# vvvwo/KSS-ICP

Measured on AMD Instinct MI355X. Metric: icp_iterations_per_sec, higher is better.
Workload: dtype f32; 1 GPU; C2: one 100000x100000 uniform-sphere pair per GPU, 50 fixed ICP iterations + fitness pass per step (exact NN + cov reduce + host 3x3 SVD), R_z(10deg), jitter 1e-3; n_src=100000, n_tgt=100000, pairs_per_gpu=1, nn_engine=cell list + brute-force fallback, nn_arithmetic=reference (no fma)

## Files before the change

### kss-icp_amd/csrc/kss_api.hip

```cpp
#pragma clang fp contract(off)

#include "kss_ctx.hpp"

extern "C" {

int kss_version(void) { return KSS_VERSION; }

const char* kss_status_string(int s) {
    switch (s) {
        case KSS_OK: return "ok";
        case KSS_ERR_ARG: return "invalid argument";
        case KSS_ERR_HIP: return "HIP runtime error";
        case KSS_ERR_NOMEM: return "out of memory";
        case KSS_ERR_NODEVICE: return "no usable GPU device";
        case KSS_ERR_CAPACITY: return "output buffer too small";
        case KSS_ERR_RCCL: return "RCCL error";
        case KSS_ERR_DEGENERATE: return "degenerate point-to-plane system";
        default: return "unknown status";
    }
}

const char* kss_last_error(const kss_ctx* ctx) { return ctx ? ctx->err.c_str() : ""; }

static int ctx_create_common(int device_id, void* stream, bool borrow, kss_ctx** out) {
// ... 5 lines not shown
    if (hipSetDevice(device_id) != hipSuccess) return KSS_ERR_NODEVICE;
    kss_ctx* c = new (std::nothrow) kss_ctx();
    if (!c) return KSS_ERR_NOMEM;
    c->device = device_id;
    if (borrow) {
        c->stream = (hipStream_t)stream;
        c->own_stream = false;
    } else {
        if (hipStreamCreateWithFlags(&c->stream, hipStreamNonBlocking) != hipSuccess) { delete c; return KSS_ERR_HIP; }
        c->own_stream = true;
    }
    kss_live_contexts().fetch_add(1);
    static std::atomic<unsigned long long> ctx_serial{0};
    c->seq = (ctx_serial.fetch_add(1) + 1ull) << 40;
    *out = c;
    return KSS_OK;
}

int kss_ctx_create(int device_id, kss_ctx** out) { return ctx_create_common(device_id, nullptr, false, out); }
int kss_ctx_create_on_stream(int device_id, void* hip_stream, kss_ctx** out) {
    return ctx_create_common(device_id, hip_stream, true, out);
}

int kss_ctx_destroy(kss_ctx* c) {
    if (!c) return KSS_ERR_ARG;
    hipSetDevice(c->device);
    hipStreamSynchronize(c->stream);
    prof_collect(c);
    for (auto& ep : c->ev_pool) { hipEventDestroy(ep.a); hipEventDestroy(ep.b); }
    c->ev_pool.clear();
    DevBuf* bufs[] = {&c->tgt4, &c->src0, &c->cur[0], &c->cur[1], &c->keys, &c->partials, &c->sums, &c->nn_work,
                      &c->red_work, &c->pair_red, &c->state, &c->cs, &c->scratch_a, &c->scratch_b, &c->scratch_c,
                      &c->stage_src, &c->stage_tgt, &c->stage_idx, &c->stage_d2, &c->stage_out, &c->g_counts, &c->g_start,
                      &c->g_cursor, &c->g_bsums, &c->g_sorted, &c->g_list, &c->g_count, &c->g_bbox, &c->g_partials, &c->g_start2, &c->g_pairs, &c->g_stamps, &c->g_pos, &c->g_nnst, &c->res_pos, &c->res_wc, &c->res_perm, &c->pack_seg, &c->reg_s, &c->reg_t, &c->reg_p, &c->reg_all, &c->reg_f, &c->reg_g, &c->oct_pts, &c->oct_cen, &c->oct_a, &c->oct_b, &c->oct_tmp, &c->pre_partials, &c->pre_state, &c->g_rowpair, &c->g_gate, &c->p2l_idx, &c->p2l_d2, &c->p2l_perm, &c->p2l_rows, &c->p2l_nrm, &c->p2l_n64, &c->trim_rows, &c->trim_state};
    for (DevBuf* b : bufs)
        if (b->p) hipFree(b->p);
    if (c->h_sums) hipHostFree(c->h_sums);
    if (c->h_seq) hipHostFree(c->h_seq);
    if (c->h_p2l) hipHostFree(c->h_p2l);
    if (c->h_box) hipHostFree(c->h_box);
    if (c->h_xf) hipHostFree(c->h_xf);
    if (c->gate_bar) hipFree(c->gate_bar);
    if (c->res_gate) hipFree(c->res_gate);
    if (c->bar_state) hipFree(c->bar_state);
    if (c->h_state) hipHostFree(c->h_state);
    for (kss_ctx* w : c->workers) kss_ctx_destroy(w);
    c->workers.clear();
    if (c->own_stream) hipStreamDestroy(c->stream);
    kss_live_contexts().fetch_sub(1);
    delete c;
    return KSS_OK;
}

int kss_ctx_synchronize(kss_ctx* c) {
    if (!c) return KSS_ERR_ARG;
    HIPCHK(c, hipStreamSynchronize(c->stream));
    return KSS_OK;
}

void* kss_ctx_stream(kss_ctx* c) { return c ? (void*)c->stream : nullptr; }

int kss_ctx_set_nn_mode(kss_ctx* c, int nn_mode) {
    if (!c || nn_mode < KSS_NN_AUTO || nn_mode > KSS_NN_GRID) return KSS_ERR_ARG;
    c->nn_mode = nn_mode;
    return KSS_OK;
}

// ... 1034 lines not shown
```

### kss-icp_amd/csrc/kss_ctx.hpp

```cpp
#pragma once
#include <dlfcn.h>
#include <hip/hip_runtime.h>

#include <algorithm>
#include <atomic>
#include <chrono>
#include <cmath>
#include <cstdio>
#include <cstdlib>
#include <cstring>
#include <mutex>
#include <string>
#include <thread>
#include <vector>

#include "kss_internal.hpp"
#include "kss_host_pool.hpp"

using namespace kss;

struct DevBuf {
    void* p = nullptr;
    size_t cap = 0;
};

struct kss_ctx {
    int device = 0;
    int cu_count = 0;
    hipStream_t stream = nullptr;
    bool own_stream = false;
    std::string err;
    int nn_mode = KSS_NN_AUTO;
    double grid_stats[8] = {0, 0, 0, 0, 0, 0, 0, 0};
    double last_setup_ms = 0, last_loop_ms = 0;
    double t_launch_us = 0, t_wait_us = 0, t_host_us = 0;
    bool timing = false;
    bool tables_staged = false;
    int64_t stats_ns = -1, stats_nt = -1;

    DevBuf tgt4, src0, cur[2], keys, partials, sums, nn_work, red_work, pair_red, state, cs, scratch_a,
        scratch_b, scratch_c, stage_src, stage_tgt, stage_idx, stage_d2, stage_out, g_counts, g_start, g_cursor,
        g_bsums, g_sorted, g_list, g_count, g_bbox, g_partials, g_start2, g_pairs, g_stamps, g_pos, g_nnst, res_pos, res_wc, res_perm, pack_seg, reg_s, reg_t, reg_p, reg_all, reg_f, reg_g, oct_pts, oct_cen, oct_a, oct_b, oct_tmp, pre_partials, pre_state, g_rowpair, g_gate;
    DevBuf p2l_idx, p2l_d2, p2l_perm, p2l_rows, p2l_nrm, p2l_n64;
    DevBuf trim_rows, trim_state;
    HostPool pool;
    std::vector<kss_ctx*> workers;
    std::vector<unsigned long long> last_stamps;
    int stamps_nblk = 0; unsigned long long stamps_seq = 0;
    std::vector<float> h_bbox;
    unsigned int* h_box = nullptr; unsigned int* h_box_dev = nullptr; size_t h_box_bytes = 0;
    unsigned box_tag = 0; int box_rows = 0;
    double evals_sum = 0.0, evals_launches = 0.0;
    void* h_sums = nullptr;  size_t h_sums_cap = 0;
    void* h_sums_dev = nullptr;
    void* h_p2l = nullptr; size_t h_p2l_cap = 0;
    void* h_p2l_dev = nullptr;
    unsigned long long* h_seq = nullptr;
    unsigned long long* h_seq_dev = nullptr;
    size_t h_seq_bytes = 0;
    struct Gated {
        int supported = -1;
        bool want_next = false;
        bool pending = false;
        bool chain = false;
        int steps_left = 0;
        int max_steps = 1;
        int slot = 0;
        unsigned long long seq = 0;
        int32_t stamp = 0;
        const void* d_in = nullptr; void* d_out = nullptr;
        bool fma = false, full = false, want_full = false; double max_d2 = 0.0;
    } gated;
    bool ws_dirty = false;
    bool defer_wait = false;
    PairState* h_xf = nullptr; PairState* h_xf_dev = nullptr;
// ... 148 lines not shown
```

### kss-icp_amd/csrc/kss_engine.hip

```cpp
#pragma clang fp contract(off)

#include <emmintrin.h>

#include "kss_ctx.hpp"

namespace kss {

static int restore_zero_at_rest(kss_ctx* c);
static bool resident_gate_available(kss_ctx* c, int npairs);

static int resident_rows_limit(kss_ctx* c) {
    if (c->cu_count <= 0) {
        hipDeviceProp_t prop;
        c->cu_count = hipGetDeviceProperties(&prop, c->device) == hipSuccess && prop.multiProcessorCount > 0 ? prop.multiProcessorCount : 1;
        (void)hipGetLastError();
    }
    return c->cu_count;
}

constexpr int PUB_PAIRS = 32;
static int ensure_pub(kss_ctx* c, int npairs = PUB_PAIRS);

struct PairGeom {
    int64_t ns, nt;
// ... 298 lines not shown
                for (int k = 0; k < 3; ++k) { if (g & 1) mx[k] = std::max(mx[k], f[k]); else mn[k] = std::min(mn[k], f[k]); }
                ++g;
                continue;
            }
            __builtin_ia32_pause();
            if ((spin & 4095) == 4095 && std::chrono::duration<double, std::milli>(std::chrono::steady_clock::now() - t0).count() > 20.0) break;
        }
        have_box = g == 2 * nbb;
        if (!have_box) { for (int k = 0; k < 3; ++k) { mn[k] = INFINITY; mx[k] = -INFINITY; } }
    }
    if (!have_box) {
        std::vector<float>& hb = c->h_bbox;
        hb.resize((size_t)nbb * 6);
        HIPCHK(c, hipMemcpyAsync(hb.data(), c->g_bbox.p, hb.size() * sizeof(float), hipMemcpyDeviceToHost, c->stream));
        HIPCHK(c, hipStreamSynchronize(c->stream));
        for (int b = 0; b < nbb; ++b)
            for (int k = 0; k < 3; ++k) { mn[k] = std::min(mn[k], hb[(size_t)b * 6 + k]); mx[k] = std::max(mx[k], hb[(size_t)b * 6 + 3 + k]); }
    }
    if (!(std::isfinite(mn[0]) && std::isfinite(mn[1]) && std::isfinite(mn[2]) && std::isfinite(mx[0]) && std::isfinite(mx[1]) && std::isfinite(mx[2])))
        return set_err(c, KSS_ERR_ARG, "non-finite target coordinates");
    GridParams gp;
    choose_cells(mn, mx, nt, gp);
    pl.gp = gp;
    const size_t ncells = (size_t)gp.gx * gp.gy * gp.gz;
    KCHK(ensure_zeroed(c, c->g_counts, 2 * ncells * sizeof(int32_t)));
    KCHK(ensure(c, c->g_start, (2 * ncells + 8) * sizeof(int32_t)));
    KCHK(ensure(c, c->g_bsums, scan_scratch_bytes((int)(2 * ncells))));
    KCHK(ensure(c, c->g_sorted, (size_t)nt * sizeof(float4)));
    KCHK(ensure(c, c->g_list, (size_t)ns * sizeof(int32_t)));
    KCHK(ensure(c, c->g_pos, (size_t)ns * sizeof(float4)));
    c->nn_have = false;
    KCHK(ensure(c, c->g_nnst, (size_t)ns * sizeof(float2)));
    KCHK(ensure_zeroed(c, c->g_count, 64));
    if (getenv("KSS_COUNTS_CHECK")) {
        HIPCHK(c, hipStreamSynchronize(c->stream));
        std::vector<int32_t> h(2 * ncells);
        HIPCHK(c, hipMemcpy(h.data(), c->g_counts.p, h.size() * sizeof(int32_t), hipMemcpyDeviceToHost));
        size_t bad = 0, first = 0;
        for (size_t k = 0; k < h.size(); ++k)
            if (h[k] != 0) { if (!bad) first = k; ++bad; }
        if (bad) {
            std::fprintf(stderr, "[kss] counts check: %zu cells x 2 (%d x %d x %d), buffer %zu bytes, %zu non-zero counters, first at %zu = %d\n", ncells,
                         gp.gx, gp.gy, gp.gz, c->g_counts.cap, bad, first, h[first]);
            return set_err(c, KSS_ERR_HIP, "cell counters not zero at rest");
        }
    }
    pl.gpairs[0].gp = gp;
    pl.gpairs[0].cell_base = 0;
    launch_grid_build_pair(c->stream, tgt, nt, (float4*)c->src0.p + g.src_base, ns, gp, (int32_t*)c->g_counts.p, (int32_t*)c->g_start.p + 1,
                           (int32_t*)c->g_bsums.p, (float4*)c->g_sorted.p, (float4*)c->cur[0].p);
    HIPCHK(c, hipGetLastError());
    c->grid_stats[0] = gp.h; c->grid_stats[1] = gp.gx; c->grid_stats[2] = gp.gy; c->grid_stats[3] = gp.gz;
    if (c->stats_ns != ns || c->stats_nt != nt) { c->grid_stats[4] = 0; c->grid_stats[5] = 0; }
    c->grid_stats[6] = ns; c->grid_stats[7] = nt;
    if (c->prof && (c->stats_ns != ns || c->stats_nt != nt)) {
        c->stats_ns = ns; c->stats_nt = nt;
        KCHK(ensure(c, c->scratch_c, 64));
        HIPCHK(c, hipMemsetAsync(c->scratch_c.p, 0, 16, c->stream));
        launch_grid_stats(c->stream, (const float4*)c->src0.p + g.src_base, ns, gp, (const int32_t*)c->g_start.p + 1, (unsigned long long*)c->scratch_c.p);
        unsigned long long hst[2] = {0, 0};
        HIPCHK(c, hipMemcpyAsync(hst, c->scratch_c.p, 16, hipMemcpyDeviceToHost, c->stream));
        HIPCHK(c, hipStreamSynchronize(c->stream));
        c->grid_stats[5] = (double)hst[0];
        c->grid_stats[4] = (double)hst[1];
    }
    return KSS_OK;
}

static int grid_setup_batch(kss_ctx* c, IcpPlan& pl) {
    if (!pl.gridb) return KSS_OK;
    const int np = pl.npairs;
    std::vector<GridPairDev>& hp = pl.gpairs;
    int64_t sum_nt = 0;
    for (int p = 0; p < np; ++p) sum_nt += pl.g[p].nt;
    ProfScope ps(c, KSS_K_GRID_BUILD);
    KCHK(ensure(c, c->g_pairs, (size_t)np * sizeof(GridPairDev)));
    KCHK(ensure(c, c->g_bbox, (size_t)np * 6 * sizeof(float)));
    HIPCHK(c, hipMemcpyAsync(c->g_pairs.p, hp.data(), (size_t)np * sizeof(GridPairDev), hipMemcpyHostToDevice, c->stream));
    launch_gridb_bbox(c->stream, (const float4*)c->tgt4.p, (const GridPairDev*)c->g_pairs.p, np, (float*)c->g_bbox.p);
    std::vector<float> hb((size_t)np * 6);
    HIPCHK(c, hipMemcpyAsync(hb.data(), c->g_bbox.p, hb.size() * sizeof(float), hipMemcpyDeviceToHost, c->stream));
    HIPCHK(c, hipStreamSynchronize(c->stream));
    int64_t cells = 0, sorted_base = 0;
// ... 1361 lines not shown
```

### kss-icp_amd/csrc/kss_grid.hip

```cpp
#pragma clang fp contract(off)

#include <hip/hip_runtime.h>

#include <cstring>

#include <rocprim/rocprim.hpp>

#include <cstdlib>

#include "kss_internal.hpp"
#include "kss_device.hpp"

namespace kss {

__global__ __launch_bounds__(256) void grid_count2_kernel(const float4* __restrict__ tgt, int nt, int nbt, const float4* __restrict__ src, int ns,
                                                          GridParams gp, int32_t* __restrict__ counts) {
    const bool is_src = (int)blockIdx.x >= nbt;
    const int i = ((int)blockIdx.x - (is_src ? nbt : 0)) * 256 + (int)threadIdx.x;
    if (i >= (is_src ? ns : nt)) return;
    const float4 p = is_src ? src[i] : tgt[i];
    const int cx = cell_coord(p.x, gp.ox, gp.inv_h, gp.gx), cy = cell_coord(p.y, gp.oy, gp.inv_h, gp.gy),
              cz = cell_coord(p.z, gp.oz, gp.inv_h, gp.gz);
    atomicAdd(&counts[(is_src ? gp.gx * gp.gy * gp.gz : 0) + (cz * gp.gy + cy) * gp.gx + cx], 1);
}

constexpr int SCAN_CHUNK = 4096;

__global__ __launch_bounds__(256) void scan_block_sums_kernel(const int32_t* __restrict__ in, int n, int32_t* __restrict__ block_sums) {
    __shared__ int sh[4];
    typedef int32_t int4u __attribute__((ext_vector_type(4), aligned(4)));
    const int base = blockIdx.x * SCAN_CHUNK;
    int s = 0;
#pragma unroll
    for (int k = 0; k < 4; ++k) {
        const int i = base + (k * 256 + (int)threadIdx.x) * 4;
        if (i + 3 < n) { const int4u v = *(const int4u*)(in + i); s += (v.x + v.y) + (v.z + v.w); }
        else { if (i < n) s += in[i]; if (i + 1 < n) s += in[i + 1]; if (i + 2 < n) s += in[i + 2]; }
    }
#pragma unroll
    for (int off = 32; off > 0; off >>= 1) s += __shfl_down(s, off, 64);
    if ((threadIdx.x & 63) == 0) sh[threadIdx.x >> 6] = s;
    __syncthreads();
    if (threadIdx.x == 0) block_sums[blockIdx.x] = sh[0] + sh[1] + sh[2] + sh[3];
}

__global__ __launch_bounds__(1024) void scan_of_block_sums_kernel(int32_t* __restrict__ block_sums, int nb) {
    __shared__ int wave_tot[16];
    const int tid = threadIdx.x, lane = tid & 63, wave = tid >> 6;
    const int per = (nb + 1023) / 1024;
    const int lo = min(tid * per, nb), hi = min(nb, lo + per);
    int s = 0;
    for (int i = lo; i < hi; ++i) s += block_sums[i];
    int incl = s;
#pragma unroll
    for (int off = 1; off < 64; off <<= 1) {
        const int v = __shfl_up(incl, off, 64);
        if (lane >= off) incl += v;
    }
    if (lane == 63) wave_tot[wave] = incl;
    __syncthreads();
    int run = incl - s;
    for (int w = 0; w < 16; ++w) run += w < wave ? wave_tot[w] : 0;
    for (int i = lo; i < hi; ++i) {
        const int v = block_sums[i];
        block_sums[i] = run;
        run += v;
    }
}

template <bool SELF>
__global__ __launch_bounds__(256) void scan_apply_kernel(const int32_t* __restrict__ in, int n, const int32_t* __restrict__ block_sums,
                                                         int32_t* __restrict__ out_start) {
    typedef int32_t int4u __attribute__((ext_vector_type(4), aligned(4)));
    __shared__ int sh_tot[4][4];
    __shared__ int sh_off[4];
    const int tid = threadIdx.x, lane = tid & 63, wave = tid >> 6;
    int offset = 0;
    if constexpr (SELF) {
        int part = 0;
        for (int b = tid; b < (int)blockIdx.x; b += 256) part += block_sums[b];
#pragma unroll
        for (int off = 32; off > 0; off >>= 1) part += __shfl_down(part, off, 64);
        if (lane == 0) sh_off[wave] = part;
    } else {
        offset = block_sums[blockIdx.x];
    }
    const int base = blockIdx.x * SCAN_CHUNK;
    int4u v[4];
    int incl[4];
#pragma unroll
    for (int k = 0; k < 4; ++k) {
        const int i = base + (k * 256 + tid) * 4;
        if (i + 3 < n) v[k] = *(const int4u*)(in + i);
        else { v[k].x = i < n ? in[i] : 0; v[k].y = i + 1 < n ? in[i + 1] : 0; v[k].z = i + 2 < n ? in[i + 2] : 0; v[k].w = 0; }
        int x = (v[k].x + v[k].y) + (v[k].z + v[k].w);
#pragma unroll
        for (int off = 1; off < 64; off <<= 1) {
            const int t = __shfl_up(x, off, 64);
            if (lane >= off) x += t;
        }
        incl[k] = x;
        if (lane == 63) sh_tot[k][wave] = x;
    }
    __syncthreads();
    if constexpr (SELF) offset = sh_off[0] + sh_off[1] + sh_off[2] + sh_off[3];
    int run = offset;
#pragma unroll
    for (int k = 0; k < 4; ++k) {
        int before = 0;
#pragma unroll
        for (int w = 0; w < 4; ++w) before += w < wave ? sh_tot[k][w] : 0;
        const int own = (v[k].x + v[k].y) + (v[k].z + v[k].w);
        const int r0 = run + before + (incl[k] - own);
        const int i = base + (k * 256 + tid) * 4;
        int4u o;
        o.x = r0; o.y = r0 + v[k].x; o.z = o.y + v[k].y; o.w = o.z + v[k].z;
        if (i + 3 < n) *(int4u*)(out_start + i) = o;
        else { if (i < n) out_start[i] = o.x; if (i + 1 < n) out_start[i + 1] = o.y; if (i + 2 < n) out_start[i + 2] = o.z; }
        if (i <= n - 1 && n - 1 <= i + 3) out_start[n] = o.x + (n - 1 >= i ? v[k].x : 0) + (n - 1 >= i + 1 ? v[k].y : 0) + (n - 1 >= i + 2 ? v[k].z : 0) + (n - 1 >= i + 3 ? v[k].w : 0);
        run += (sh_tot[k][0] + sh_tot[k][1]) + (sh_tot[k][2] + sh_tot[k][3]);
    }
}

using BigScanConfig = rocprim::scan_config<256, 64, rocprim::block_load_method::block_load_transpose, rocprim::block_store_method::block_store_transpose,
                                           rocprim::block_scan_algorithm::reduce_then_scan>;

size_t scan_scratch_bytes(int n) {
    size_t bytes = 0;
    if (rocprim::inclusive_scan<BigScanConfig>(nullptr, bytes, (const int32_t*)nullptr, (int32_t*)nullptr, (size_t)n, rocprim::plus<int32_t>(), (hipStream_t)0) != hipSuccess) bytes = 0;
    return std::max<size_t>(bytes, ((size_t)(n + SCAN_CHUNK - 1) / SCAN_CHUNK + 1) * sizeof(int32_t)) + 256;
}

static void launch_scan(hipStream_t st, const int32_t* d_counts, int ncells, int32_t* d_start, int32_t* d_scratch) {
    static const bool lib = getenv("KSS_SCAN_LIB") != nullptr;
    if (lib && ncells > 1024 * SCAN_CHUNK) {
        size_t bytes = 0;
        if (rocprim::inclusive_scan<BigScanConfig>(nullptr, bytes, d_counts, d_start + 1, (size_t)ncells, rocprim::plus<int32_t>(), st) == hipSuccess) {
            hipMemsetAsync(d_start, 0, sizeof(int32_t), st);
            if (rocprim::inclusive_scan<BigScanConfig>((void*)d_scratch, bytes, d_counts, d_start + 1, (size_t)ncells, rocprim::plus<int32_t>(), st) == hipSuccess) return;
        }
        (void)hipGetLastError();
    }
    int32_t* d_block_sums = d_scratch;
    const int nb = (ncells + SCAN_CHUNK - 1) / SCAN_CHUNK;
    hipLaunchKernelGGL(scan_block_sums_kernel, dim3(nb), dim3(256), 0, st, d_counts, ncells, d_block_sums);
    if (nb <= 1024) {
        hipLaunchKernelGGL(scan_apply_kernel<true>, dim3(nb), dim3(256), 0, st, d_counts, ncells, d_block_sums, d_start);
    } else {
        hipLaunchKernelGGL(scan_of_block_sums_kernel, dim3(1), dim3(1024), 0, st, d_block_sums, nb);
        hipLaunchKernelGGL(scan_apply_kernel<false>, dim3(nb), dim3(256), 0, st, d_counts, ncells, d_block_sums, d_start);
    }
}

__global__ __launch_bounds__(256) void grid_scatter2_kernel(const float4* __restrict__ tgt, int nt, int nbt, const float4* __restrict__ src, int ns,
                                                            GridParams gp, int32_t* __restrict__ counts, const int32_t* __restrict__ start,
                                                            float4* __restrict__ sorted, float4* __restrict__ src_tmp) {
    const bool is_src = (int)blockIdx.x >= nbt;
    const int i = ((int)blockIdx.x - (is_src ? nbt : 0)) * 256 + (int)threadIdx.x;
    if (i >= (is_src ? ns : nt)) return;
    float4 p = is_src ? src[i] : tgt[i];
    const int cx = cell_coord(p.x, gp.ox, gp.inv_h, gp.gx), cy = cell_coord(p.y, gp.oy, gp.inv_h, gp.gy),
              cz = cell_coord(p.z, gp.oz, gp.inv_h, gp.gz);
    const int cell = (is_src ? gp.gx * gp.gy * gp.gz : 0) + (cz * gp.gy + cy) * gp.gx + cx;
    const int pos = start[cell] + atomicSub(&counts[cell], 1) - 1 - (is_src ? nt : 0);
    p.w = __int_as_float(i);
    (is_src ? src_tmp : sorted)[pos] = p;
}

template <bool FMA>
__device__ __forceinline__ unsigned long long point_key(const float4 p, float qx, float qy, float qz) {
    const float dx = qx - p.x, dy = qy - p.y, dz = qz - p.z;
    float d;
    if constexpr (FMA) d = __builtin_fmaf(dx, dx, __builtin_fmaf(dy, dy, dz * dz));
    else d = (dx * dx + dy * dy) + dz * dz;
    return ((unsigned long long)__float_as_uint(d) << 32) | (unsigned long long)(unsigned)__float_as_int(p.w);
}

template <bool FMA>
__device__ __forceinline__ void scan_range(const float4* __restrict__ sorted, int lo, int hi, float qx, float qy, float qz,
                                           unsigned long long& key, int& kpos) {
    for (int k = lo; k < hi; k += 4) {
        const int k1 = min(k + 1, hi - 1), k2 = min(k + 2, hi - 1), k3 = min(k + 3, hi - 1);
        const float4 p0 = sorted[k], p1 = sorted[k1], p2 = sorted[k2], p3 = sorted[k3];
        const unsigned long long e0 = point_key<FMA>(p0, qx, qy, qz), e1 = point_key<FMA>(p1, qx, qy, qz),
                                 e2 = point_key<FMA>(p2, qx, qy, qz), e3 = point_key<FMA>(p3, qx, qy, qz);
        if (e0 < key) { key = e0; kpos = k; }
        if (e1 < key) { key = e1; kpos = k1; }
        if (e2 < key) { key = e2; kpos = k2; }
        if (e3 < key) { key = e3; kpos = k3; }
    }
}

typedef int32_t int4u __attribute__((ext_vector_type(4), aligned(4)));

template <bool FMA, int BS, int U>
__device__ __forceinline__ int block_walk(const GridParams& gp, const int32_t* __restrict__ cell_start, const float4* __restrict__ sorted,
                                          float qx, float qy, float qz, int cx, int cy, int cz, float rho, unsigned rowmask,
// ... 96 lines not shown
            if constexpr (TWO) at[j] = f >= total ? last : f < n0 ? lo0 + f : lo1 + (f - n0);
            else at[j] = min(lo0 + f, hi0 - 1);
        }
#pragma unroll
        for (int j = 0; j < U; ++j) pt[j] = sorted[at[j]];
#pragma unroll
        for (int j = 0; j < U; ++j) {
            const unsigned long long kk = point_key<FMA>(pt[j], qx, qy, qz);
            if (kk < key) { key = kk; kpos = at[j]; }
            const float dd = e + j < total ? __uint_as_float((unsigned)(kk >> 32)) : __builtin_inff();
            m2 = __builtin_amdgcn_fmed3f(m1, m2, dd);
            m1 = fminf(m1, dd);
        }
    }
}

__global__ __launch_bounds__(256) void grid_rank_fix_kernel(const float4* __restrict__ tmp, int n, GridParams gp,
                                                            const int32_t* __restrict__ start , int shift,
                                                            float4* __restrict__ out) {
    const int j = blockIdx.x * blockDim.x + threadIdx.x;
    if (j >= n) return;
    const float4 p = tmp[j];
    const int cx = cell_coord(p.x, gp.ox, gp.inv_h, gp.gx), cy = cell_coord(p.y, gp.oy, gp.inv_h, gp.gy),
              cz = cell_coord(p.z, gp.oz, gp.inv_h, gp.gz);
    const int c = (cz * gp.gy + cy) * gp.gx + cx;
    const int lo = start[c] - shift, hi = start[c + 1] - shift;
    const int me = __float_as_int(p.w);
    int rank = 0;
    for (int k = lo; k < hi; ++k) rank += __float_as_int(tmp[k].w) < me ? 1 : 0;
    out[lo + rank] = p;
}

void launch_grid_build_pair(hipStream_t st, const float4* d_tgt, int nt, float4* d_src, int ns, const GridParams& gp, int32_t* d_counts,
                            int32_t* d_start, int32_t* d_block_sums, float4* d_sorted, float4* d_tmp) {
    const int ncells = gp.gx * gp.gy * gp.gz;
    const int nbt = (nt + 255) / 256, nbs = (ns + 255) / 256;
    hipLaunchKernelGGL(grid_count2_kernel, dim3(nbt + nbs), dim3(256), 0, st, d_tgt, nt, nbt, (const float4*)d_src, ns, gp, d_counts);
    launch_scan(st, d_counts, 2 * ncells, d_start, d_block_sums);
    hipLaunchKernelGGL(grid_scatter2_kernel, dim3(nbt + nbs), dim3(256), 0, st, d_tgt, nt, nbt, (const float4*)d_src, ns, gp, d_counts,
                       (const int32_t*)d_start, d_sorted, d_tmp);
    hipLaunchKernelGGL(grid_rank_fix_kernel, dim3(nbs), dim3(256), 0, st, (const float4*)d_tmp, ns, gp, (const int32_t*)d_start + ncells, nt,
                       d_src);
}

struct SkipOut {
    unsigned long long key;
    int kpos;
    float rho;
    float acc;
    bool walker;
};
template <bool FMA>
__device__ __forceinline__ SkipOut skip_test(bool qok, float qx, float qy, float qz, float pold_x, float pold_y, float pold_z, const float4& prevp,
                                             const float2& st, bool chained_k, float skin_frac, float h) {
    SkipOut o;
    o.key = ~0ull; o.kpos = -1; o.rho = __builtin_inff(); o.acc = 0.f; o.walker = false;
    if (!qok) return o;
    o.walker = true;
    if (__float_as_uint(prevp.w) != ~0u) {
        o.key = point_key<FMA>(prevp, qx, qy, qz);
        o.kpos = -2;
        const float d0 = __uint_as_float((unsigned)(o.key >> 32));
        const float mx = qx - pold_x, my = qy - pold_y, mz = qz - pold_z;
        const float moved = __builtin_amdgcn_sqrtf((mx * mx + my * my) + mz * mz);
        const float acc = (st.y + moved) * 1.00001f;
        const float room = st.x - acc;
        if (chained_k && skin_frac >= 0.f && room > 1e-7f && (room * room) * 0.99999f > d0) {
            o.walker = false;
            o.acc = acc;
        } else {
            const float skin = fmaxf(skin_frac, 0.f) * h, grown = __builtin_amdgcn_sqrtf(d0) + skin;
            o.rho = !chained_k || moved * 4.f <= skin ? fmaxf(d0, grown * grown) : d0;
        }
// ... 149 lines not shown
            } else {
                a.keys[io] = ~0ull;
                const int ls = atomicAdd(a.list_count, 1);
                a.list[ls] = io;
                wfell = true;
            }
            a.nn_win[io] = make_float4(ww.x, ww.y, ww.z, __uint_as_float(whave ? (unsigned)wkey : ~0u));
            a.nn_state[io] = make_float2(wfell ? 0.f : bnew, 0.f);
            s_ent[WK_X][owner] = __float_as_uint(ww.x); s_ent[WK_Y][owner] = __float_as_uint(ww.y); s_ent[WK_Z][owner] = __float_as_uint(ww.z);
            s_ent[WK_IDX][owner] = (unsigned)wkey; s_ent[WK_D2][owner] = (unsigned)(wkey >> 32);
            s_ent[WK_FL][owner] = (whave ? 1u : 0u) | (wfell ? 2u : 0u);
            s_ent[WK_R][owner] = __float_as_uint(wfell ? 0.f : bnew);
        }
        KSS_STAMP(8);
        if (a.stamps) {
            int evs = evl, mx = evl;
#pragma unroll
            for (int m = 32; m > 0; m >>= 1) { evs += __shfl_xor(evs, m, 64); mx = max(mx, __shfl_xor(mx, m, 64)); }
            if (lane == 0) {
                atomicAdd(&a.stamps[(size_t)blockIdx.x * 16 + 10], (unsigned long long)evs);
                atomicAdd(&a.stamps[(size_t)blockIdx.x * 16 + 11], (unsigned long long)(((mx + 7) / 8) * 8 * 64));
            }
        }
    }
#undef KSS_STAMP
}

#ifndef KSS_BATCH_WAVES
#define KSS_BATCH_WAVES 6
#endif
#ifndef KSS_SINGLE_WAVES
#define KSS_SINGLE_WAVES 1
#endif
template <bool FMA, bool FULL, bool BATCH, bool SEARCH, bool CHAIN>
__global__ __launch_bounds__(PASS_BS, BATCH ? KSS_BATCH_WAVES : KSS_SINGLE_WAVES) void grid_pass_kernel(const PassArgs a) {
    static_assert(!CHAIN || (!BATCH && SEARCH), "chained launches: single pair, search passes");
#define KSS_STAMP(k) do { if (a.stamps && threadIdx.x == 0) a.stamps[(size_t)blockIdx.x * 16 + (k)] = __builtin_amdgcn_s_memrealtime(); } while (0)
    KSS_STAMP(0);
    constexpr int BS = PASS_BS;
    const int per_xcd = (int)gridDim.x / 8;
    const int w = ((int)blockIdx.x % 8) * per_xcd + (int)blockIdx.x / 8;
    if (w >= a.total_rows) return;
    int pi = 0;
    if constexpr (BATCH) pi = a.row_pair[w];
    const GridPairDev pr = BATCH ? a.pairs[pi] : a.pair0;
    PairState ps = a.ps0;
    if constexpr (BATCH) {
        ps = a.state[pi];
        if (!ps.active) return;
    }
    const GridParams& gp = pr.gp;
    const int32_t* __restrict__ cs = a.cell_start + pr.cell_base;
    const float4* __restrict__ sorted = a.sorted;
    constexpr int WQ = 256;
    __shared__ int2 rowq[9][WQ];
    __shared__ double shw[BS / 64][NSUMS];
    __shared__ int s_last;
    __shared__ int sh_ps[16];
    __shared__ int s_nwalk;
    __shared__ unsigned s_ent[7][BS];
    __shared__ unsigned short s_wl[BS];
    enum { WK_X, WK_Y, WK_Z, WK_IDX, WK_D2, WK_R, WK_POS, WK_FL = WK_POS, WK_COLS };
    static_assert(sizeof(PairState) == 64, "the gated launch reads the transform record as 16 dwords");
    double (*shf)[NSUMS] = reinterpret_cast<double (*)[NSUMS]>(&rowq[0][0]);
    static_assert(sizeof(double) * PASS_FG * NSUMS <= sizeof(int2) * 9 * WQ, "shf must fit inside rowq");

    const int local = (w - pr.row_base) * BS + (int)threadIdx.x;
    const bool valid = local < pr.src_n;
    const int i = pr.src_base + local;
    const int lane = threadIdx.x & 63, wave = threadIdx.x >> 6;
    bool have = false, fell_back = false;
    float qx = 0.f, qy = 0.f, qz = 0.f, d2 = 0.f;
    float4 win = make_float4(0.f, 0.f, 0.f, 0.f);
    float4 p = make_float4(0.f, 0.f, 0.f, 0.f), prevp = make_float4(0.f, 0.f, 0.f, __uint_as_float(~0u));
    float2 st = make_float2(0.f, 0.f);
    if (valid) {
        p = SEARCH ? a.src_in[i] : a.src_out[i];
        if (!SEARCH || a.use_prev) { prevp = a.nn_win[i]; st = a.nn_state[i]; }
    }
    for (int step = 0;; ++step) {
    const bool last_step = !CHAIN || step + 1 >= a.chain_len;
    const unsigned long long seq_k = a.seq + (unsigned long long)step;
    const int gate_k = a.gate_seq != 0 ? a.gate_seq + step : 0;
    unsigned int* const gate_ptr = a.gate_dev + 32 * ((a.gate_slot + step) & 1);
    float4* const src_out_k = (step & 1) ? a.src_alt : a.src_out;
    const bool last_known = a.chained == 2 && ps.pad[0] > 0;
    const bool chained_k = step > 0 || a.chained == 1 || last_known;
    const bool has_prev = __float_as_uint(prevp.w) != ~0u;
    if constexpr (SEARCH) {
        __syncthreads();
        if (threadIdx.x == 0) s_nwalk = 0;
        __syncthreads();
    }
    KSS_STAMP(13);
    if constexpr (!BATCH && SEARCH) {
        if (gate_k != 0) {
            typedef unsigned int u32x4 __attribute__((ext_vector_type(4)));
            if (a.state && w == 0 && threadIdx.x < 16) {
                const int* w32 = reinterpret_cast<const int*>(a.state);
                int v = 0, n = 0;
                bool ok = true;
                for (;;) {
                    v = __hip_atomic_load(w32 + threadIdx.x, __ATOMIC_RELAXED, __HIP_MEMORY_SCOPE_SYSTEM);
                    if (__shfl(v, 15, 64) == gate_k) break;
                    __builtin_amdgcn_s_sleep(1);
                    if (++n > a.gate_polls / 2) { ok = false; break; }
                }
                if (ok) {
                    const int g = threadIdx.x;
                    const int w0 = __shfl(v, min(3 * g, 15), 64), w1 = __shfl(v, min(3 * g + 1, 15), 64), w2 = __shfl(v, min(3 * g + 2, 15), 64);
                    if (g < 5) {
                        u32x4 o;
                        o.x = (unsigned)w0; o.y = (unsigned)w1; o.z = (unsigned)w2; o.w = (unsigned)gate_k + kss_mix3(o.x, o.y, o.z);
                        unsigned int* dst = gate_ptr + 4 * g;
                        asm volatile("global_store_dwordx4 %0, %1, off sc1" ::"v"(dst), "v"(o) : "memory");
                    }
                }
            }
            if (threadIdx.x < 8) {
                const unsigned int* src = gate_ptr + 4 * min((int)threadIdx.x, 4);
                u32x4 v;
                int n = 0;
                bool ok = true;
                for (;;) {
                    asm volatile("global_load_dwordx4 %0, %1, off sc0 sc1\n\ts_waitcnt vmcnt(0)" : "=&v"(v) : "v"(src) : "memory");
                    if (__builtin_amdgcn_ballot_w64(v.w - kss_mix3(v.x, v.y, v.z) == (unsigned)gate_k) == 0xffull) break;
                    __builtin_amdgcn_s_sleep(1);
                    if (++n > a.gate_polls) { ok = false; break; }
// ... 44 lines not shown
        bool walker = false;
        float acc_keep = 0.f;
        {
            const bool qok = valid && (qx - qx) == 0.f && (qy - qy) == 0.f && (qz - qz) == 0.f;
            const SkipOut so = skip_test<FMA>(qok, qx, qy, qz, pold_x, pold_y, pold_z, prevp, st, chained_k, a.skin, gp.h);
            walker = so.walker;
            key = so.key;
            acc_keep = so.acc;
            unsigned fl = 0u;
            if (qok && !walker) {
                fl = 1u;
                a.nn_state[i] = make_float2(st.x, so.acc);
            } else if (valid && !qok) {
                a.nn_win[i] = make_float4(0.f, 0.f, 0.f, __uint_as_float(~0u));
                a.nn_state[i] = make_float2(0.f, 0.f);
            }
            const float4 c4 = walker ? make_float4(qx, qy, qz, 0.f) : prevp;
            s_ent[WK_X][threadIdx.x] = __float_as_uint(c4.x); s_ent[WK_Y][threadIdx.x] = __float_as_uint(c4.y); s_ent[WK_Z][threadIdx.x] = __float_as_uint(c4.z);
            s_ent[WK_IDX][threadIdx.x] = (unsigned)key; s_ent[WK_D2][threadIdx.x] = (unsigned)(key >> 32);
            s_ent[WK_POS][threadIdx.x] = walker ? (unsigned)so.kpos : fl;
            s_ent[WK_R][threadIdx.x] = __float_as_uint(so.rho);
        }
        const unsigned long long wm = __builtin_amdgcn_ballot_w64(walker);
        if (wm != 0ull) {
            int base = 0;
            if (lane == 0) base = atomicAdd(&s_nwalk, (int)__builtin_popcountll(wm));
            base = __builtin_amdgcn_readfirstlane(base);
            if (walker) s_wl[base + (int)__builtin_amdgcn_mbcnt_hi((unsigned)(wm >> 32), __builtin_amdgcn_mbcnt_lo((unsigned)wm, 0u))] = (unsigned short)threadIdx.x;
        }
        KSS_STAMP(14);
        __syncthreads();
        const int nwalk = s_nwalk;
        if (a.stamps && threadIdx.x == 0) a.stamps[(size_t)blockIdx.x * 16 + 12] = (unsigned long long)nwalk;
        serve_walkers<FMA, BATCH, WQ, BS, BATCH ? 4 : 8>(a, pr, cs, sorted, w, nwalk, rowq, s_ent, s_wl);
        KSS_STAMP(15);
        __syncthreads();
        {
            const unsigned fl = s_ent[WK_FL][threadIdx.x];
            have = (fl & 1u) != 0u; fell_back = (fl & 2u) != 0u;
            win = make_float4(__uint_as_float(s_ent[WK_X][threadIdx.x]), __uint_as_float(s_ent[WK_Y][threadIdx.x]), __uint_as_float(s_ent[WK_Z][threadIdx.x]), 0.f);
            key = ((unsigned long long)s_ent[WK_D2][threadIdx.x] << 32) | (unsigned long long)s_ent[WK_IDX][threadIdx.x];
            if (CHAIN && !last_step) {
                if (walker) {
                    prevp = make_float4(win.x, win.y, win.z, __uint_as_float(have ? (unsigned)key : ~0u));
                    st = make_float2(__uint_as_float(s_ent[WK_R][threadIdx.x]), 0.f);
                } else if (have) {
                    st.y = acc_keep;
                } else {
                    prevp.w = __uint_as_float(~0u);
                    st = make_float2(0.f, 0.f);
                }
            }
        }
        if constexpr (BATCH) {
            p = make_float4(0.f, 0.f, 0.f, 0.f);
            if (valid) p = src_out_k[i];
            qx = p.x; qy = p.y; qz = p.z;
        }
    }
    if (valid && have) {
        d2 = __uint_as_float((unsigned)(key >> 32));
        const int oi = __float_as_int(p.w);
        if (a.idx_out) a.idx_out[oi] = (int)(unsigned)(key & 0xffffffffull);
        if (a.d2_out) a.d2_out[oi] = d2;
    }
    KSS_STAMP(1);

// ... 473 lines not shown
    const int i = blockIdx.x * blockDim.x + threadIdx.x;
    unsigned long long ev = 0, occ = 0;
    if (i < ns) {
        const float4 p = src[i];
        const int cx = cell_coord(p.x, gp.ox, gp.inv_h, gp.gx), cy = cell_coord(p.y, gp.oy, gp.inv_h, gp.gy),
                  cz = cell_coord(p.z, gp.oz, gp.inv_h, gp.gz);
        const int x0 = max(cx - 1, 0), x1 = min(cx + 1, gp.gx - 1);
        for (int t = 0; t < 9; ++t) {
            const int z = cz + t / 3 - 1, y = cy + t % 3 - 1;
            if (z < 0 || z >= gp.gz || y < 0 || y >= gp.gy) continue;
            const int row = (z * gp.gy + y) * gp.gx;
            ev += (unsigned long long)(cell_start[row + x1 + 1] - cell_start[row + x0]);
        }
    }
    const int ncells = gp.gx * gp.gy * gp.gz;
    for (int c = blockIdx.x * blockDim.x + threadIdx.x; c < ncells; c += gridDim.x * blockDim.x)
        occ += cell_start[c + 1] > cell_start[c] ? 1 : 0;
    atomicAdd(&out[0], ev);
    atomicAdd(&out[1], occ);
}

void launch_grid_stats(hipStream_t st, const float4* d_src, int ns, const GridParams& gp, const int32_t* d_cell_start,
                       unsigned long long* d_out) {
    hipLaunchKernelGGL(grid_stats_kernel, dim3((ns + 255) / 256), dim3(256), 0, st, d_src, ns, gp, d_cell_start, d_out);
}

int grid_pass_blocks(int total_rows) { return (total_rows + 7) / 8 * 8; }

void launch_grid_pass(hipStream_t st, bool fma, bool full, bool batch, bool search, const PassArgs& a) {
    if (a.total_rows <= 0) return;
    const dim3 grid(grid_pass_blocks(a.total_rows)), block(PASS_BS);
#define KSS_PASS(F, U, B, S) hipLaunchKernelGGL((grid_pass_kernel<F, U, B, S, false>), grid, block, 0, st, a)
#define KSS_CHAIN(F, U) hipLaunchKernelGGL((grid_pass_kernel<F, U, false, true, true>), grid, block, 0, st, a)
    if (!search) {
        if (fma) KSS_PASS(true, true, false, false); else KSS_PASS(false, true, false, false);
    } else if (batch) {
        static const bool old_form = getenv("KSS_BATCH_OLD") != nullptr;
        if (old_form) {
            if (fma) { if (full) KSS_PASS(true, true, true, true); else KSS_PASS(true, false, true, true); }
            else     { if (full) KSS_PASS(false, true, true, true); else KSS_PASS(false, false, true, true); }
        } else {
            const dim3 block2(256);
#define KSS_PASSB(F, U, Q) hipLaunchKernelGGL((gridb_pass_kernel<F, U, Q>), grid, block2, 0, st, a)
            if (!a.use_prev) {
                if (fma) { if (full) KSS_PASSB(true, true, 256); else KSS_PASSB(true, false, 256); }
                else     { if (full) KSS_PASSB(false, true, 256); else KSS_PASSB(false, false, 256); }
            } else {
                if (fma) { if (full) KSS_PASSB(true, true, 128); else KSS_PASSB(true, false, 128); }
                else     { if (full) KSS_PASSB(false, true, 128); else KSS_PASSB(false, false, 128); }
            }
#undef KSS_PASSB
        }
        if (a.defer_pairs) hipLaunchKernelGGL(gridb_finalize_kernel, dim3(a.defer_pairs), dim3(256), 0, st, a, full ? 1 : 0);
    } else if (a.chain_len > 1) {
        if (fma) { if (full) KSS_CHAIN(true, true); else KSS_CHAIN(true, false); }
        else     { if (full) KSS_CHAIN(false, true); else KSS_CHAIN(false, false); }
    } else {
        if (fma) { if (full) KSS_PASS(true, true, false, true); else KSS_PASS(true, false, false, true); }
        else     { if (full) KSS_PASS(false, true, false, true); else KSS_PASS(false, false, false, true); }
    }
#undef KSS_PASS
#undef KSS_CHAIN
}

}
```

### kss-icp_amd/csrc/kss_internal.hpp

```cpp
#pragma once
#include <hip/hip_runtime.h>

#include <algorithm>
#include <cfloat>
#include <cmath>
#include <cstdint>
#include <functional>
#include <string>
#include <vector>

#include "../../include/kssicp.h"
#include "kss_host_math.hpp"

namespace kss {

struct alignas(16) PairState {
    float m[12];
    int32_t active;
    int32_t apply;
    int32_t pad[2];
};

struct alignas(16) NNWork {
    int32_t pair;
// ... 150 lines not shown
    }
}
inline bool oct_adopt(OctBox& b, const float* p) {
    const float minValue = FLT_EPSILON;
    for (;;) {
        bool up[3], any = false;
        for (int k = 0; k < 3; ++k) { up[k] = p[k] >= b.max[k]; any = any || up[k] || p[k] < b.min[k]; }
        if (!any) return true;
        if (b.depth >= 21) return false;
        double side = (double)(1u << b.depth) * b.res;
        for (int k = 0; k < 3; ++k) if (!up[k]) b.min[k] -= side;
        ++b.depth;
        side = (double)(1u << b.depth) * b.res - minValue;
        for (int k = 0; k < 3; ++k) b.max[k] = b.min[k] + side;
    }
}

void launch_pack_f3_to_f4(hipStream_t st, const float* d_in, int64_t n, float4* d_out, int64_t n_pad, bool sentinel);
void launch_pack_f64_to_f4(hipStream_t st, const double* d_in, int64_t n, float4* d_out, int64_t n_pad, bool sentinel);
void launch_empty(hipStream_t st);
int pack_pair_bbox_rows(int64_t nt_pad);
void launch_pack_pair(hipStream_t st, int dtype, const void* d_tgt, int64_t nt, float4* d_tgt_out, int64_t nt_pad, float* d_bbox_partial,
                      const void* d_src, int64_t ns, float4* d_src_out, unsigned int* d_box_host, unsigned box_tag);
void launch_pack_batch(hipStream_t st, const void* d_in, int dtype, const PackSeg* d_seg, int nseg, int64_t total_out, float4* d_out);

void launch_nn_sweep(hipStream_t st, int S, bool fma, const NNWork* d_work, int n_work,
                     const PairState* d_state, const float4* d_src_in, float4* d_src_out,
                     const float4* d_tgt4, unsigned long long* d_keys);

void launch_nn_sweep_list(hipStream_t st, int S, bool fma, const NNWork* d_work, int n_work,
                          const PairState* d_state, float4* d_src_cur, const float4* d_tgt4,
                          unsigned long long* d_keys, const int32_t* d_list, const int32_t* d_count);
void launch_grid_build_pair(hipStream_t st, const float4* d_tgt, int nt, float4* d_src, int ns, const GridParams& gp, int32_t* d_counts,
                            int32_t* d_start, int32_t* d_block_sums, float4* d_sorted, float4* d_tmp);
size_t scan_scratch_bytes(int n);
int grid_pass_blocks(int total_rows);
void launch_grid_pass(hipStream_t st, bool fma, bool full, bool batch, bool search, const PassArgs& a);
void launch_gridb_bbox(hipStream_t st, const float4* d_tgt, const GridPairDev* d_pairs, int npairs, float* d_bbox);
void launch_gridb_build_targets(hipStream_t st, const float4* d_tgt, int total_tgt_pad, const GridPairDev* d_pairs, int npairs,
                                int total_cells, int32_t* d_counts, int32_t* d_start, int32_t* d_block_sums, float4* d_sorted);
void launch_gridb_sort_sources(hipStream_t st, const float4* d_src, int total_src, const GridPairDev* d_pairs, int npairs,
                               int total_cells, int32_t* d_counts, int32_t* d_start, int32_t* d_block_sums, float4* d_tmp, float4* d_out);
int gridb_lds_max_cells(bool half);
bool launch_gridb_build_lds(hipStream_t st, const float4* d_tgt4, float4* d_src, float4* d_tmp, const GridPairDev* d_pairs, int npairs,
                            int32_t* d_cell_start, float4* d_sorted, int max_cells, bool half);
void launch_grid_stats(hipStream_t st, const float4* d_src, int ns, const GridParams& gp, const int32_t* d_cell_start,
                       unsigned long long* d_out );

void launch_corr_reduce(hipStream_t st, const RedWork* d_work, int n_work, const PairState* d_state,
                        const float4* d_src, const float4* d_tgt4, const unsigned long long* d_keys,
                        double max_d2, double* d_partials, int32_t* d_idx_out, float* d_d2_out, int index_in_w);
void launch_corr_reduce_publish(hipStream_t st, const RedWork* d_work, int n_work, const PairState* d_state,
                                const float4* d_src, const float4* d_tgt4, const unsigned long long* d_keys,
                                double max_d2, Granule* d_rows, int32_t* d_idx_out, float* d_d2_out, int index_in_w,
                                const PairRed* d_pair_red, unsigned long long* d_pub, unsigned long long seq);
size_t cand_pass_lds_bytes(int nt_pad);
int cand_pass_blocks_per_pair(int64_t ns);
bool launch_cand_pass(hipStream_t st, bool fma, int npairs, const PairState* d_state, const float4* d_src_in, float4* d_src_out, const float4* d_tgt,
                      int nt_pad, int ns, double max_d2, Granule* d_rows, unsigned long long* d_pub, unsigned long long seq,
                      int32_t* d_idx_out, float* d_d2_out);
constexpr int CAND_TPW = 4;
struct CandArgs {
    const float4* src0;
    const float4* tgt;
    int32_t nt_pad, ns;
    int32_t bpp, wpp, tpw;
    double max_d2;
// ... 78 lines not shown
```

Before: 81460 iterations/s.

## Record per-point slots in grid count and widen first search pass

Grid build now stores each point's atomicAdd return value as its slot within its cell during counting. Scatter then computes the position from start plus slot instead of doing a second atomicSub, and the scan zeroes the counts in place. Separately, the first ungated, non-chained search pass gets a wide variant with a larger row queue, a wider walker fan-out, and the gate logic skipped. Both are enabled by default and add an extra int buffer plus more kernel instantiations.

```diff
diff --git a/kss-icp_amd/csrc/kss_api.hip b/kss-icp_amd/csrc/kss_api.hip
--- a/kss-icp_amd/csrc/kss_api.hip
+++ b/kss-icp_amd/csrc/kss_api.hip
@@ -61,7 +61,7 @@
     DevBuf* bufs[] = {&c->tgt4, &c->src0, &c->cur[0], &c->cur[1], &c->keys, &c->partials, &c->sums, &c->nn_work,
                       &c->red_work, &c->pair_red, &c->state, &c->cs, &c->scratch_a, &c->scratch_b, &c->scratch_c,
                       &c->stage_src, &c->stage_tgt, &c->stage_idx, &c->stage_d2, &c->stage_out, &c->g_counts, &c->g_start,
-                      &c->g_cursor, &c->g_bsums, &c->g_sorted, &c->g_list, &c->g_count, &c->g_bbox, &c->g_partials, &c->g_start2, &c->g_pairs, &c->g_stamps, &c->g_pos, &c->g_nnst, &c->res_pos, &c->res_wc, &c->res_perm, &c->pack_seg, &c->reg_s, &c->reg_t, &c->reg_p, &c->reg_all, &c->reg_f, &c->reg_g, &c->oct_pts, &c->oct_cen, &c->oct_a, &c->oct_b, &c->oct_tmp, &c->pre_partials, &c->pre_state, &c->g_rowpair, &c->g_gate, &c->p2l_idx, &c->p2l_d2, &c->p2l_perm, &c->p2l_rows, &c->p2l_nrm, &c->p2l_n64, &c->trim_rows, &c->trim_state};
+                      &c->g_cursor, &c->g_bsums, &c->g_sorted, &c->g_list, &c->g_count, &c->g_bbox, &c->g_partials, &c->g_start2, &c->g_pairs, &c->g_stamps, &c->g_pos, &c->g_nnst, &c->res_pos, &c->res_wc, &c->res_perm, &c->pack_seg, &c->reg_s, &c->reg_t, &c->reg_p, &c->reg_all, &c->reg_f, &c->reg_g, &c->oct_pts, &c->oct_cen, &c->oct_a, &c->oct_b, &c->oct_tmp, &c->pre_partials, &c->pre_state, &c->g_rowpair, &c->g_gate, &c->g_slots, &c->p2l_idx, &c->p2l_d2, &c->p2l_perm, &c->p2l_rows, &c->p2l_nrm, &c->p2l_n64, &c->trim_rows, &c->trim_state};
     for (DevBuf* b : bufs)
         if (b->p) hipFree(b->p);
     if (c->h_sums) hipHostFree(c->h_sums);
diff --git a/kss-icp_amd/csrc/kss_ctx.hpp b/kss-icp_amd/csrc/kss_ctx.hpp
--- a/kss-icp_amd/csrc/kss_ctx.hpp
+++ b/kss-icp_amd/csrc/kss_ctx.hpp
@@ -40,7 +40,7 @@
 
     DevBuf tgt4, src0, cur[2], keys, partials, sums, nn_work, red_work, pair_red, state, cs, scratch_a,
         scratch_b, scratch_c, stage_src, stage_tgt, stage_idx, stage_d2, stage_out, g_counts, g_start, g_cursor,
-        g_bsums, g_sorted, g_list, g_count, g_bbox, g_partials, g_start2, g_pairs, g_stamps, g_pos, g_nnst, res_pos, res_wc, res_perm, pack_seg, reg_s, reg_t, reg_p, reg_all, reg_f, reg_g, oct_pts, oct_cen, oct_a, oct_b, oct_tmp, pre_partials, pre_state, g_rowpair, g_gate;
+        g_bsums, g_sorted, g_list, g_count, g_bbox, g_partials, g_start2, g_pairs, g_stamps, g_pos, g_nnst, res_pos, res_wc, res_perm, pack_seg, reg_s, reg_t, reg_p, reg_all, reg_f, reg_g, oct_pts, oct_cen, oct_a, oct_b, oct_tmp, pre_partials, pre_state, g_rowpair, g_gate, g_slots;
     DevBuf p2l_idx, p2l_d2, p2l_perm, p2l_rows, p2l_nrm, p2l_n64;
     DevBuf trim_rows, trim_state;
     HostPool pool;
diff --git a/kss-icp_amd/csrc/kss_engine.hip b/kss-icp_amd/csrc/kss_engine.hip
--- a/kss-icp_amd/csrc/kss_engine.hip
+++ b/kss-icp_amd/csrc/kss_engine.hip
@@ -354,6 +354,8 @@
     c->nn_have = false;
     KCHK(ensure(c, c->g_nnst, (size_t)ns * sizeof(float2)));
     KCHK(ensure_zeroed(c, c->g_count, 64));
+    static const bool build_slots = getenv("KSS_BUILD_SLOTS") == nullptr || atoi(getenv("KSS_BUILD_SLOTS")) != 0;
+    if (build_slots) KCHK(ensure(c, c->g_slots, ((size_t)nt + (size_t)ns) * sizeof(int32_t)));
     if (getenv("KSS_COUNTS_CHECK")) {
         HIPCHK(c, hipStreamSynchronize(c->stream));
         std::vector<int32_t> h(2 * ncells);
@@ -370,7 +372,7 @@
     pl.gpairs[0].gp = gp;
     pl.gpairs[0].cell_base = 0;
     launch_grid_build_pair(c->stream, tgt, nt, (float4*)c->src0.p + g.src_base, ns, gp, (int32_t*)c->g_counts.p, (int32_t*)c->g_start.p + 1,
-                           (int32_t*)c->g_bsums.p, (float4*)c->g_sorted.p, (float4*)c->cur[0].p);
+                           (int32_t*)c->g_bsums.p, (float4*)c->g_sorted.p, (float4*)c->cur[0].p, build_slots ? (int32_t*)c->g_slots.p : nullptr);
     HIPCHK(c, hipGetLastError());
     c->grid_stats[0] = gp.h; c->grid_stats[1] = gp.gx; c->grid_stats[2] = gp.gy; c->grid_stats[3] = gp.gz;
     if (c->stats_ns != ns || c->stats_nt != nt) { c->grid_stats[4] = 0; c->grid_stats[5] = 0; }
diff --git a/kss-icp_amd/csrc/kss_grid.hip b/kss-icp_amd/csrc/kss_grid.hip
--- a/kss-icp_amd/csrc/kss_grid.hip
+++ b/kss-icp_amd/csrc/kss_grid.hip
@@ -13,15 +13,18 @@
 
 namespace kss {
 
+template <bool SLOTS>
 __global__ __launch_bounds__(256) void grid_count2_kernel(const float4* __restrict__ tgt, int nt, int nbt, const float4* __restrict__ src, int ns,
-                                                          GridParams gp, int32_t* __restrict__ counts) {
+                                                          GridParams gp, int32_t* __restrict__ counts, int32_t* __restrict__ slots) {
     const bool is_src = (int)blockIdx.x >= nbt;
     const int i = ((int)blockIdx.x - (is_src ? nbt : 0)) * 256 + (int)threadIdx.x;
     if (i >= (is_src ? ns : nt)) return;
     const float4 p = is_src ? src[i] : tgt[i];
     const int cx = cell_coord(p.x, gp.ox, gp.inv_h, gp.gx), cy = cell_coord(p.y, gp.oy, gp.inv_h, gp.gy),
               cz = cell_coord(p.z, gp.oz, gp.inv_h, gp.gz);
-    atomicAdd(&counts[(is_src ? gp.gx * gp.gy * gp.gz : 0) + (cz * gp.gy + cy) * gp.gx + cx], 1);
+    int32_t* const cnt = &counts[(is_src ? gp.gx * gp.gy * gp.gz : 0) + (cz * gp.gy + cy) * gp.gx + cx];
+    if constexpr (SLOTS) slots[(is_src ? nt : 0) + i] = atomicAdd(cnt, 1);
+    else atomicAdd(cnt, 1);
 }
 
 constexpr int SCAN_CHUNK = 4096;
@@ -68,7 +71,7 @@
     }
 }
 
-template <bool SELF>
+template <bool SELF, bool ZERO = false>
 __global__ __launch_bounds__(256) void scan_apply_kernel(const int32_t* __restrict__ in, int n, const int32_t* __restrict__ block_sums,
                                                          int32_t* __restrict__ out_start) {
     typedef int32_t int4u __attribute__((ext_vector_type(4), aligned(4)));
@@ -93,6 +96,12 @@
         const int i = base + (k * 256 + tid) * 4;
         if (i + 3 < n) v[k] = *(const int4u*)(in + i);
         else { v[k].x = i < n ? in[i] : 0; v[k].y = i + 1 < n ? in[i + 1] : 0; v[k].z = i + 2 < n ? in[i + 2] : 0; v[k].w = 0; }
+        if constexpr (ZERO) {
+            int32_t* const z = const_cast<int32_t*>(in);
+            const int4u zero = {0, 0, 0, 0};
+            if (i + 3 < n) *(int4u*)(z + i) = zero;
+            else { if (i < n) z[i] = 0; if (i + 1 < n) z[i + 1] = 0; if (i + 2 < n) z[i + 2] = 0; }
+        }
         int x = (v[k].x + v[k].y) + (v[k].z + v[k].w);
 #pragma unroll
         for (int off = 1; off < 64; off <<= 1) {
@@ -131,13 +140,16 @@
     return std::max<size_t>(bytes, ((size_t)(n + SCAN_CHUNK - 1) / SCAN_CHUNK + 1) * sizeof(int32_t)) + 256;
 }
 
-static void launch_scan(hipStream_t st, const int32_t* d_counts, int ncells, int32_t* d_start, int32_t* d_scratch) {
+static void launch_scan(hipStream_t st, const int32_t* d_counts, int ncells, int32_t* d_start, int32_t* d_scratch, bool zero = false) {
     static const bool lib = getenv("KSS_SCAN_LIB") != nullptr;
     if (lib && ncells > 1024 * SCAN_CHUNK) {
         size_t bytes = 0;
         if (rocprim::inclusive_scan<BigScanConfig>(nullptr, bytes, d_counts, d_start + 1, (size_t)ncells, rocprim::plus<int32_t>(), st) == hipSuccess) {
             hipMemsetAsync(d_start, 0, sizeof(int32_t), st);
-            if (rocprim::inclusive_scan<BigScanConfig>((void*)d_scratch, bytes, d_counts, d_start + 1, (size_t)ncells, rocprim::plus<int32_t>(), st) == hipSuccess) return;
+            if (rocprim::inclusive_scan<BigScanConfig>((void*)d_scratch, bytes, d_counts, d_start + 1, (size_t)ncells, rocprim::plus<int32_t>(), st) == hipSuccess) {
+                if (zero) hipMemsetAsync(const_cast<int32_t*>(d_counts), 0, (size_t)ncells * sizeof(int32_t), st);
+                return;
+            }
         }
         (void)hipGetLastError();
     }
@@ -145,16 +157,19 @@
     const int nb = (ncells + SCAN_CHUNK - 1) / SCAN_CHUNK;
     hipLaunchKernelGGL(scan_block_sums_kernel, dim3(nb), dim3(256), 0, st, d_counts, ncells, d_block_sums);
     if (nb <= 1024) {
-        hipLaunchKernelGGL(scan_apply_kernel<true>, dim3(nb), dim3(256), 0, st, d_counts, ncells, d_block_sums, d_start);
+        if (zero) hipLaunchKernelGGL((scan_apply_kernel<true, true>), dim3(nb), dim3(256), 0, st, d_counts, ncells, d_block_sums, d_start);
+        else hipLaunchKernelGGL(scan_apply_kernel<true>, dim3(nb), dim3(256), 0, st, d_counts, ncells, d_block_sums, d_start);
     } else {
         hipLaunchKernelGGL(scan_of_block_sums_kernel, dim3(1), dim3(1024), 0, st, d_block_sums, nb);
-        hipLaunchKernelGGL(scan_apply_kernel<false>, dim3(nb), dim3(256), 0, st, d_counts, ncells, d_block_sums, d_start);
-    }
-}
-
+        if (zero) hipLaunchKernelGGL((scan_apply_kernel<false, true>), dim3(nb), dim3(256), 0, st, d_counts, ncells, d_block_sums, d_start);
+        else hipLaunchKernelGGL(scan_apply_kernel<false>, dim3(nb), dim3(256), 0, st, d_counts, ncells, d_block_sums, d_start);
+    }
+}
+
+template <bool SLOTS>
 __global__ __launch_bounds__(256) void grid_scatter2_kernel(const float4* __restrict__ tgt, int nt, int nbt, const float4* __restrict__ src, int ns,
                                                             GridParams gp, int32_t* __restrict__ counts, const int32_t* __restrict__ start,
-                                                            float4* __restrict__ sorted, float4* __restrict__ src_tmp) {
+                                                            const int32_t* __restrict__ slots, float4* __restrict__ sorted, float4* __restrict__ src_tmp) {
     const bool is_src = (int)blockIdx.x >= nbt;
     const int i = ((int)blockIdx.x - (is_src ? nbt : 0)) * 256 + (int)threadIdx.x;
     if (i >= (is_src ? ns : nt)) return;
@@ -162,7 +177,9 @@
     const int cx = cell_coord(p.x, gp.ox, gp.inv_h, gp.gx), cy = cell_coord(p.y, gp.oy, gp.inv_h, gp.gy),
               cz = cell_coord(p.z, gp.oz, gp.inv_h, gp.gz);
     const int cell = (is_src ? gp.gx * gp.gy * gp.gz : 0) + (cz * gp.gy + cy) * gp.gx + cx;
-    const int pos = start[cell] + atomicSub(&counts[cell], 1) - 1 - (is_src ? nt : 0);
+    int pos;
+    if constexpr (SLOTS) pos = start[cell] + slots[(is_src ? nt : 0) + i] - (is_src ? nt : 0);
+    else pos = start[cell] + atomicSub(&counts[cell], 1) - 1 - (is_src ? nt : 0);
     p.w = __int_as_float(i);
     (is_src ? src_tmp : sorted)[pos] = p;
 }
@@ -325,13 +342,20 @@
 }
 
 void launch_grid_build_pair(hipStream_t st, const float4* d_tgt, int nt, float4* d_src, int ns, const GridParams& gp, int32_t* d_counts,
-                            int32_t* d_start, int32_t* d_block_sums, float4* d_sorted, float4* d_tmp) {
+                            int32_t* d_start, int32_t* d_block_sums, float4* d_sorted, float4* d_tmp, int32_t* d_slots) {
     const int ncells = gp.gx * gp.gy * gp.gz;
     const int nbt = (nt + 255) / 256, nbs = (ns + 255) / 256;
-    hipLaunchKernelGGL(grid_count2_kernel, dim3(nbt + nbs), dim3(256), 0, st, d_tgt, nt, nbt, (const float4*)d_src, ns, gp, d_counts);
-    launch_scan(st, d_counts, 2 * ncells, d_start, d_block_sums);
-    hipLaunchKernelGGL(grid_scatter2_kernel, dim3(nbt + nbs), dim3(256), 0, st, d_tgt, nt, nbt, (const float4*)d_src, ns, gp, d_counts,
-                       (const int32_t*)d_start, d_sorted, d_tmp);
+    if (d_slots) {
+        hipLaunchKernelGGL(grid_count2_kernel<true>, dim3(nbt + nbs), dim3(256), 0, st, d_tgt, nt, nbt, (const float4*)d_src, ns, gp, d_counts, d_slots);
+        launch_scan(st, d_counts, 2 * ncells, d_start, d_block_sums, true);
+        hipLaunchKernelGGL(grid_scatter2_kernel<true>, dim3(nbt + nbs), dim3(256), 0, st, d_tgt, nt, nbt, (const float4*)d_src, ns, gp, d_counts,
+                           (const int32_t*)d_start, (const int32_t*)d_slots, d_sorted, d_tmp);
+    } else {
+        hipLaunchKernelGGL(grid_count2_kernel<false>, dim3(nbt + nbs), dim3(256), 0, st, d_tgt, nt, nbt, (const float4*)d_src, ns, gp, d_counts, d_slots);
+        launch_scan(st, d_counts, 2 * ncells, d_start, d_block_sums);
+        hipLaunchKernelGGL(grid_scatter2_kernel<false>, dim3(nbt + nbs), dim3(256), 0, st, d_tgt, nt, nbt, (const float4*)d_src, ns, gp, d_counts,
+                           (const int32_t*)d_start, (const int32_t*)d_slots, d_sorted, d_tmp);
+    }
     hipLaunchKernelGGL(grid_rank_fix_kernel, dim3(nbs), dim3(256), 0, st, (const float4*)d_tmp, ns, gp, (const int32_t*)d_start + ncells, nt,
                        d_src);
 }
@@ -547,9 +571,10 @@
 #ifndef KSS_SINGLE_WAVES
 #define KSS_SINGLE_WAVES 1
 #endif
-template <bool FMA, bool FULL, bool BATCH, bool SEARCH, bool CHAIN>
+template <bool FMA, bool FULL, bool BATCH, bool SEARCH, bool CHAIN, bool WIDE = false>
 __global__ __launch_bounds__(PASS_BS, BATCH ? KSS_BATCH_WAVES : KSS_SINGLE_WAVES) void grid_pass_kernel(const PassArgs a) {
     static_assert(!CHAIN || (!BATCH && SEARCH), "chained launches: single pair, search passes");
+    static_assert(!WIDE || (!BATCH && SEARCH && !CHAIN), "the first-pass form: single pair, plain search launches");
 #define KSS_STAMP(k) do { if (a.stamps && threadIdx.x == 0) a.stamps[(size_t)blockIdx.x * 16 + (k)] = __builtin_amdgcn_s_memrealtime(); } while (0)
     KSS_STAMP(0);
     constexpr int BS = PASS_BS;
@@ -567,7 +592,7 @@
     const GridParams& gp = pr.gp;
     const int32_t* __restrict__ cs = a.cell_start + pr.cell_base;
     const float4* __restrict__ sorted = a.sorted;
-    constexpr int WQ = 256;
+    constexpr int WQ = WIDE ? BS : 256;
     __shared__ int2 rowq[9][WQ];
     __shared__ double shw[BS / 64][NSUMS];
     __shared__ int s_last;
@@ -608,7 +633,7 @@
         __syncthreads();
     }
     KSS_STAMP(13);
-    if constexpr (!BATCH && SEARCH) {
+    if constexpr (!BATCH && SEARCH && !WIDE) {
         if (gate_k != 0) {
             typedef unsigned int u32x4 __attribute__((ext_vector_type(4)));
             if (a.state && w == 0 && threadIdx.x < 16) {
@@ -719,7 +744,7 @@
         __syncthreads();
         const int nwalk = s_nwalk;
         if (a.stamps && threadIdx.x == 0) a.stamps[(size_t)blockIdx.x * 16 + 12] = (unsigned long long)nwalk;
-        serve_walkers<FMA, BATCH, WQ, BS, BATCH ? 4 : 8>(a, pr, cs, sorted, w, nwalk, rowq, s_ent, s_wl);
+        serve_walkers<FMA, BATCH, WQ, BS, BATCH ? 4 : WIDE ? 16 : 8>(a, pr, cs, sorted, w, nwalk, rowq, s_ent, s_wl);
         KSS_STAMP(15);
         __syncthreads();
         {
@@ -1259,6 +1284,8 @@
     const dim3 grid(grid_pass_blocks(a.total_rows)), block(PASS_BS);
 #define KSS_PASS(F, U, B, S) hipLaunchKernelGGL((grid_pass_kernel<F, U, B, S, false>), grid, block, 0, st, a)
 #define KSS_CHAIN(F, U) hipLaunchKernelGGL((grid_pass_kernel<F, U, false, true, true>), grid, block, 0, st, a)
+#define KSS_WIDE(F, U) hipLaunchKernelGGL((grid_pass_kernel<F, U, false, true, false, true>), grid, block, 0, st, a)
+    static const bool first_wide = getenv("KSS_FIRST_WIDE") == nullptr || atoi(getenv("KSS_FIRST_WIDE")) != 0;
     if (!search) {
         if (fma) KSS_PASS(true, true, false, false); else KSS_PASS(false, true, false, false);
     } else if (batch) {
@@ -1282,11 +1309,15 @@
     } else if (a.chain_len > 1) {
         if (fma) { if (full) KSS_CHAIN(true, true); else KSS_CHAIN(true, false); }
         else     { if (full) KSS_CHAIN(false, true); else KSS_CHAIN(false, false); }
+    } else if (first_wide && !a.use_prev && a.gate_seq == 0) {
+        if (fma) { if (full) KSS_WIDE(true, true); else KSS_WIDE(true, false); }
+        else     { if (full) KSS_WIDE(false, true); else KSS_WIDE(false, false); }
     } else {
         if (fma) { if (full) KSS_PASS(true, true, false, true); else KSS_PASS(true, false, false, true); }
         else     { if (full) KSS_PASS(false, true, false, true); else KSS_PASS(false, false, false, true); }
     }
 #undef KSS_PASS
+#undef KSS_WIDE
 #undef KSS_CHAIN
 }
 
diff --git a/kss-icp_amd/csrc/kss_internal.hpp b/kss-icp_amd/csrc/kss_internal.hpp
--- a/kss-icp_amd/csrc/kss_internal.hpp
+++ b/kss-icp_amd/csrc/kss_internal.hpp
@@ -206,7 +206,7 @@
                           const PairState* d_state, float4* d_src_cur, const float4* d_tgt4,
                           unsigned long long* d_keys, const int32_t* d_list, const int32_t* d_count);
 void launch_grid_build_pair(hipStream_t st, const float4* d_tgt, int nt, float4* d_src, int ns, const GridParams& gp, int32_t* d_counts,
-                            int32_t* d_start, int32_t* d_block_sums, float4* d_sorted, float4* d_tmp);
+                            int32_t* d_start, int32_t* d_block_sums, float4* d_sorted, float4* d_tmp, int32_t* d_slots);
 size_t scan_scratch_bytes(int n);
 int grid_pass_blocks(int total_rows);
 void launch_grid_pass(hipStream_t st, bool fma, bool full, bool batch, bool search, const PassArgs& a);
```

Result: faster. 83300 iterations/s (median of 6 runs) (+2.2%).
